# dizgotti/ouroboros-network

Measured on AMD Instinct MI355X. Metric: TPraos header verifies/sec (VRF+KES+Ed25519) at 1/2/4/8 MI355X; Ed25519 ver/s, higher is better.
Workload: dtype u32/u64 (GF(2^255-19) int limbs)

## Files before the change

### ouroboros-network_amd/csrc/devhost_vrfkey.hip

```cpp
#define OURO_NI_LINKAGE static
#include <algorithm>
#include <cstring>
#include <vector>

#include "lane_items.h"
#include "tpraos.h"
#include "vrfkey_ws.h"

using namespace ouro;

namespace {
const int32_t* host_btab() {
  static std::vector<int32_t> tab = [] {
    std::vector<int32_t> t(kBTabWords);
    build_btab(t.data());
    return t;
  }();
  return tab.data();
}
const int32_t* host_ubtab() {
  static std::vector<int32_t> tab = [] {
    std::vector<int32_t> t(kUBTabWords);
    build_ubtab(t.data());
    return t;
  }();
  return tab.data();
}
struct Lane {
  std::vector<int32_t> buf;
  Slot s;
  Lane() : buf(slot_region_words(1, kLaneWords) + 4, 0) {
    s = Slot{reinterpret_cast<int32_t*>((reinterpret_cast<uintptr_t>(buf.data()) + 15) & ~uintptr_t(15))};
  }
};
void encode_result(uint8_t* out, Slot lane) {
  const ge_p2 U = dsm_result(lane);
  uint32_t enc[8];
  ge_encode_with_inv(enc, U.X, U.Y, fe_invert(U.Z));
  memcpy(out, enc, 32);
}
}

extern "C" {

void dh_vrfkey_params(int* width, int* windows, int* entries, size_t* tab_words,
                      size_t* base_words, size_t* min_per_key) {
  *width = kYW;
  *windows = kYWindows;
  *entries = kYKeyEntries;
  *tab_words = kYKeyWords;
  *base_words = kYBaseWords;
  *min_per_key = kVrfKeyMinPerKey;
}
int dh_vrfkey_build(const uint8_t* pk, int32_t* tab, int32_t* base) {
  uint32_t p[8];
  bytes_to_words8(p, pk);
  const bool ok = vrfkey_base(p, base);
  for (int j = 0; j < kYWindows; j++) vrfkey_fill(base, tab, j);
  return ok ? 1 : 0;
}
void dh_vrfkey_u(uint8_t* out, const int32_t* tab, const uint8_t* c16, const uint8_t* s32) {
  alignas(16) uint8_t proof[80] = {0};
  memcpy(proof + 32, c16, 16);
  memcpy(proof + 48, s32, 32);
  ouro_tpraos_batch b{};
  b.n = 1;
  b.eta_proof = proof;
  Lane lane;
  std::vector<int32_t> res(kResWords + 4, 0);
  hdr_u_shared(b, 0, false, true, lane.s, Slot{res.data()}, host_ubtab(), tab);
  encode_result(out, lane.s);
}
int dh_vrfkey_u_inline(uint8_t* out, const uint8_t* pk, const uint8_t* c16, const uint8_t* s32) {
  uint32_t p[8], pi[20] = {0};
  bytes_to_words8(p, pk);
  memcpy(pi + 8, c16, 16);
  memcpy(pi + 12, s32, 32);
  Lane lane;
  const bool ok = vrf_u_core(p, pi, true, 2, lane.s, host_btab());
  encode_result(out, lane.s);
  return ok ? 1 : 0;
}
int dh_tpraos_verify_shared(const ouro_tpraos_batch* b, const int32_t* tab, int key_ok,
                            uint8_t* verdict, uint8_t* beta_eta, uint8_t* beta_leader) {
  Lane lane;
  std::vector<int32_t> rr(kResWords + 4, 0);
  const Slot r{rr.data()};
  const uint32_t opts = batch_opts(*b);
  for (size_t i = 0; i < b->n; i++) {
    std::fill(rr.begin(), rr.end(), 0);
    for (int core = 0; core < kHdrCores; core++) {
      if (core == kCoreUe || core == kCoreUl)
        hdr_u_shared(*b, i, core == kCoreUl, key_ok != 0, lane.s, r, host_ubtab(), tab);
      else
        hdr_core(*b, i, opts, core, lane.s, r, host_btab());
    }
    hdr_finish_item(*b, i, opts, r, lane.s, verdict, beta_eta, beta_leader);
  }
  return 0;
}
size_t dh_vrfkey_layout(size_t n, size_t budget, size_t* out7) {
  const VrfKeyLayout L = vrfkey_layout(n, kYKeyBytes, budget);
  const size_t v[7] = {L.kmax, L.cap, L.off_rep, L.off_uniq, L.off_kidx, L.off_flag, L.group_bytes};
  memcpy(out7, v, sizeof v);
  return L.table_bytes;
}

int dh_lt_u_table(int nkeys, const uint8_t* keys, int n, const uint32_t* kidx,
                  const uint8_t* proofs, int stride, uint32_t* out) {
  if (nkeys <= 0 || n <= 0 || stride <= 0 || !keys || !kidx || !proofs || !out) return -1;
  std::vector<int32_t> tabs((size_t)nkeys * kYKeyWords), base(kYBaseWords);
  std::vector<uint8_t> flag(nkeys);
  for (int k = 0; k < nkeys; k++)
    flag[k] = (uint8_t)dh_vrfkey_build(keys + 32 * (size_t)k, tabs.data() + (size_t)k * kYKeyWords,
                                       base.data());
  ouro_tpraos_batch b{};
  b.n = (size_t)n;
  b.eta_proof = proofs;
  for (int i = 0; i < n; i++) {
    if (kidx[i] >= (uint32_t)nkeys) return -1;
    Lane lane;
    std::vector<int32_t> res(kResWords + 4, 0);
    lt::u_table_item(b, (size_t)i, flag[kidx[i]] != 0, out + (size_t)i * lt::kChainOut, lane.s,
                     Slot{res.data()}, host_ubtab(), tabs.data() + (size_t)kidx[i] * kYKeyWords);
  }
  return 0;
}
}
```

### ouroboros-network_amd/csrc/verify.h

```cpp
#pragma once
#include <vector>

#include "blake2b.h"
#include "ge25519.h"
#include "lattice.h"
#include "modinv.h"
#include "sc25519.h"
#include "sha512.h"

namespace ouro {

constexpr int kCachedWords = 40;
constexpr int kTabEntries = 8;
constexpr int kTabWords = kTabEntries * kCachedWords;
constexpr int kSlotTab1 = 0;
constexpr int kSlotTab2 = kTabWords;
constexpr int kSlotTab3 = 2 * kTabWords;
constexpr int kSlotA1 = 3 * kTabWords;
constexpr int kSlotA2 = kSlotA1 + 8;
constexpr int kSlotB = kSlotA2 + 8;
constexpr int kSlotCarry = kSlotB + 8;
constexpr int kSlotOut = kSlotCarry + 8;
constexpr int kLaneWords = kSlotOut + 36;

#ifndef OURO_SLOT_GROUP
#define OURO_SLOT_GROUP 1
#endif
constexpr int kSlotGroup = OURO_SLOT_GROUP;
constexpr int kChunkStride = 4 * kSlotGroup;
struct Slot {
  int32_t* p;
  OURO_FI Slot operator+(int w) const {
    OURO_TRK(if (w & 3) ouro_trk_violation();)
    return Slot{p + (w >> 2) * kChunkStride};
  }
  OURO_FI Slot chunks(int k) const { return Slot{p + k * kChunkStride}; }
  OURO_FI int32_t* word(int w) const { return p + (w >> 2) * kChunkStride + (w & 3); }
  OURO_FI int4* chunk(int k) const { return reinterpret_cast<int4*>(p + k * kChunkStride); }
};
OURO_FI Slot slot_of(int32_t* base, size_t s, int slot_words) {
  return Slot{base + (s / kSlotGroup) * (size_t)kSlotGroup * slot_words + (s % kSlotGroup) * 4};
}
constexpr size_t slot_region_words(size_t n, int slot_words) {
  return (n + kSlotGroup - 1) / kSlotGroup * kSlotGroup * (size_t)slot_words;
}

#ifndef OURO_BW
#define OURO_BW 16
#endif
constexpr int kBW = OURO_BW;
constexpr int kBStride = kBW / 4;
constexpr bool kBSplitRecode = (128 % kBW) != 0;
constexpr int kBDigitsHalf = kBSplitRecode ? (128 + kBW) / kBW : 128 / kBW;
constexpr int kBTabEntries = 1 << (kBW - 1);
constexpr int kNielsWords = 32;
constexpr size_t kBTabWords = 2 * (size_t)kBTabEntries * kNielsWords;

OURO_FI void st_fe(Slot p, const fe& f) {
  stg4(p.chunk(0), make_int4(f.v[0], f.v[1], f.v[2], f.v[3]));
  stg4(p.chunk(1), make_int4(f.v[4], f.v[5], f.v[6], f.v[7]));
  stg2(p.chunk(2), make_int2(f.v[8], f.v[9]));
  OURO_TRK(ouro_trk_store(p.p, f.b));
}
OURO_FI fe ld_fe(Slot p) {
  const int4 a = ldg4(p.chunk(0)), b = ldg4(p.chunk(1));
  const int2 c = ldg2(p.chunk(2));
  fe f = fe_make(a.x, a.y, a.z, a.w, b.x, b.y, b.z, b.w, c.x, c.y);
  OURO_TRK(ouro_trk_load(p.p, f.b));
  return f;
}
OURO_FI fe ld_fe_w2(const int32_t* base, int w0, int stride) {
  int2 q[5];
#pragma unroll
  for (int j = 0; j < 5; j++) {
    const int w = w0 + 2 * j;
    q[j] = ldg2(base + (w >> 2) * stride + (w & 3));
  }
  return fe_make(q[0].x, q[0].y, q[1].x, q[1].y, q[2].x, q[2].y, q[3].x, q[3].y, q[4].x, q[4].y);
}
OURO_FI void st_cached(Slot p, const ge_cached& c) {
  const uint32_t* s[4] = {c.YplusX.v, c.YminusX.v, c.Z2.v, c.T2d.v};
  int32_t w[40];
#pragma unroll
  for (int k = 0; k < 4; k++)
#pragma unroll
    for (int i = 0; i < 10; i++) w[10 * k + i] = s[k][i];
#pragma unroll
  for (int i = 0; i < 10; i++)
    stg4(p.chunk(i), make_int4(w[4 * i], w[4 * i + 1], w[4 * i + 2], w[4 * i + 3]));
  OURO_TRK(ouro_trk_store(p.word(0), c.YplusX.b); ouro_trk_store(p.word(10), c.YminusX.b);
           ouro_trk_store(p.word(20), c.Z2.b); ouro_trk_store(p.word(30), c.T2d.b);)
}
OURO_FI ge_cached ld_cached(Slot p) {
  int32_t w[40];
#pragma unroll
  for (int i = 0; i < 10; i++) {
    int4 v = ldg4(p.chunk(i));
    w[4 * i] = v.x; w[4 * i + 1] = v.y; w[4 * i + 2] = v.z; w[4 * i + 3] = v.w;
  }
  ge_cached c;
#pragma unroll
  for (int i = 0; i < 10; i++) {
    c.YplusX.v[i] = w[i];
    c.YminusX.v[i] = w[10 + i];
    c.Z2.v[i] = w[20 + i];
    c.T2d.v[i] = w[30 + i];
  }
  OURO_TRK(ouro_trk_load(p.word(0), c.YplusX.b); ouro_trk_load(p.word(10), c.YminusX.b);
           ouro_trk_load(p.word(20), c.Z2.b); ouro_trk_load(p.word(30), c.T2d.b);)
  return c;
}
#ifndef OURO_TAB_PACK
#define OURO_TAB_PACK 1
#endif
constexpr int kPackedWords = 32;
constexpr int kLaneEntryWords = OURO_TAB_PACK ? kPackedWords : kCachedWords;
OURO_FI void fe_pack256(uint32_t w[8], const fe& f) {
  OURO_TRK(for (int i = 0; i < 10; i++) trk_check(f.b[i] < (1ull << 28));)
  uint32_t h[10];
#pragma unroll
  for (int i = 0; i < 10; i++) h[i] = f.v[i];
  uint32_t c = h[9] >> 25;
  h[9] &= limb_mask(9);
  h[0] += 19 * c;
#pragma unroll
  for (int i = 0; i < 9; i++) {
    c = h[i] >> limb_bits(i);
    h[i] &= limb_mask(i);
    h[i + 1] += c;
  }
  w[0] = h[0] | (h[1] << 26);
  w[1] = (h[1] >> 6) | (h[2] << 19);
  w[2] = (h[2] >> 13) | (h[3] << 13);
  w[3] = (h[3] >> 19) | (h[4] << 6);
  w[4] = h[5] | (h[6] << 25);
  w[5] = (h[6] >> 7) | (h[7] << 19);
  w[6] = (h[7] >> 13) | (h[8] << 12);
  w[7] = (h[8] >> 20) | (h[9] << 6);
}
OURO_FI fe fe_unpack256(const uint32_t w[8]) {
  fe h;
  h.v[0] = w[0] & 0x3ffffff;
  h.v[1] = ((w[0] >> 26) | (w[1] << 6)) & 0x1ffffff;
  h.v[2] = ((w[1] >> 19) | (w[2] << 13)) & 0x3ffffff;
  h.v[3] = ((w[2] >> 13) | (w[3] << 19)) & 0x1ffffff;
  h.v[4] = (w[3] >> 6) & 0x3ffffff;
  h.v[5] = w[4] & 0x1ffffff;
  h.v[6] = ((w[4] >> 25) | (w[5] << 7)) & 0x3ffffff;
  h.v[7] = ((w[5] >> 19) | (w[6] << 13)) & 0x1ffffff;
  h.v[8] = ((w[6] >> 12) | (w[7] << 20)) & 0x3ffffff;
  h.v[9] = w[7] >> 6;
  OURO_TRK(for (int i = 0; i < 9; i++) h.b[i] = limb_mask(i); h.b[9] = (1u << 26) - 1;)
  return h;
}
OURO_FI void st_cached_packed(Slot p, const ge_cached& c) {
  const fe* s[4] = {&c.YplusX, &c.YminusX, &c.Z2, &c.T2d};
#pragma unroll
  for (int k = 0; k < 4; k++) {
    uint32_t w[8];
    fe_pack256(w, *s[k]);
    stg4(p.chunk(2 * k), make_int4((int)w[0], (int)w[1], (int)w[2], (int)w[3]));
    stg4(p.chunk(2 * k + 1), make_int4((int)w[4], (int)w[5], (int)w[6], (int)w[7]));
  }
}
OURO_FI ge_cached ld_cached_packed(Slot p) {
  fe f[4];
#pragma unroll
  for (int k = 0; k < 4; k++) {
    const int4 a = ldg4(p.chunk(2 * k)), b = ldg4(p.chunk(2 * k + 1));
    const uint32_t w[8] = {(uint32_t)a.x, (uint32_t)a.y, (uint32_t)a.z, (uint32_t)a.w,
                           (uint32_t)b.x, (uint32_t)b.y, (uint32_t)b.z, (uint32_t)b.w};
    f[k] = fe_unpack256(w);
  }
  return ge_cached{f[0], f[1], f[2], f[3]};
}
OURO_FI void st_entry(Slot p, const ge_cached& c, bool quad) {
  if (OURO_TAB_PACK && !quad)
    st_cached_packed(p, c);
  else
    st_cached(p, c);
}
OURO_FI ge_niels ld_niels(const int32_t* p) {
  int32_t w[32];
#pragma unroll
  for (int i = 0; i < 8; i++) {
    int4 v = ldg4(p + 4 * i);
    w[4 * i] = v.x; w[4 * i + 1] = v.y; w[4 * i + 2] = v.z; w[4 * i + 3] = v.w;
  }
  ge_niels n;
#pragma unroll
  for (int i = 0; i < 10; i++) {
    n.yplusx.v[i] = w[i];
    n.yminusx.v[i] = w[10 + i];
    n.xy2d.v[i] = w[20 + i];
  }
  OURO_TRK(ouro_trk_load(p, n.yplusx.b); ouro_trk_load(p + 10, n.yminusx.b);
           ouro_trk_load(p + 20, n.xy2d.b);)
  return n;
}
OURO_FI void st_words8(Slot p, const uint32_t w[8]) {
  stg4(p.chunk(0), make_int4((int)w[0], (int)w[1], (int)w[2], (int)w[3]));
  stg4(p.chunk(1), make_int4((int)w[4], (int)w[5], (int)w[6], (int)w[7]));
}
OURO_FI void ld_words8(uint32_t w[8], Slot p) {
  const int4 a = ldg4(p.chunk(0)), b = ldg4(p.chunk(1));
  w[0] = a.x; w[1] = a.y; w[2] = a.z; w[3] = a.w;
  w[4] = b.x; w[5] = b.y; w[6] = b.z; w[7] = b.w;
}
OURO_FI uint64_t ld_carry(Slot lane, int k) { return ldg8(lane.word(kSlotCarry + 2 * k)); }
OURO_FI void st_carry(Slot lane, int k, uint64_t c) { stg8(lane.word(kSlotCarry + 2 * k), c); }
struct SlotTail {
  Slot s;
  OURO_FI uint32_t tail(uint32_t q) const {
    return ((uint32_t)ldg1(s.word((int)(q >> 2))) >> (8 * (q & 3))) & 0xffu;
  }
};

OURO_HD inline void build_table(Slot tab, const ge_p3& P, bool quad = false) {
  const int ec = (quad ? kCachedWords : kLaneEntryWords) / 4;
  ge_cached c1 = ge_p3_to_cached(P);
  st_entry(tab, c1, quad);
  ge_p3 Pk = quad ? ge_p1p1_to_p3_quad(ge_p2_dbl_quad(ge_p3_to_p2(P)))
                  : ge_p1p1_to_p3(ge_p3_dbl(P));
  st_entry(tab.chunks(ec), ge_p3_to_cached(Pk), quad);
#pragma unroll 1
  for (int k = 2; k < kTabEntries; k++) {
    Pk = quad ? ge_p1p1_to_p3_quad(ge_add_cached_quad(Pk, c1, false))
              : ge_p1p1_to_p3(ge_add_cached(Pk, c1, false));
    st_entry(tab.chunks(k * ec), ge_p3_to_cached(Pk), quad);
  }
}

OURO_FI uint64_t sc_recode_b(const uint32_t s[8]) {
  if constexpr (!kBSplitRecode) {
    return sc_recode_carries<kBW, 2 * kBDigitsHalf>(s);
  } else {
  uint64_t mask = 0;
#pragma unroll
  for (int h = 0; h < 2; h++) {
    uint32_t c = 0;
#pragma unroll
    for (int k = 0; k < kBDigitsHalf; k++) {
      const int rel = kBW * k, bit = 128 * h + rel;
      const int w = bit >> 5, sh = bit & 31;
      const uint64_t two = (uint64_t)s[w] | ((w + 1 < 8 ? (uint64_t)s[w + 1] : 0ull) << 32);
      uint32_t v = (uint32_t)(two >> sh) & ((1u << kBW) - 1);
      if (128 - rel < kBW) v &= (1u << (128 - rel)) - 1;
      mask |= (uint64_t)c << (kBDigitsHalf * h + k);
      c = (v + c) > (1u << (kBW - 1)) ? 1u : 0u;
    }
  }
  return mask;
  }
}

OURO_FI void ss_shr5(uint32_t w[5], int bits) {
#pragma unroll
  for (int i = 0; i < 4; i++) w[i] = (w[i] >> bits) | (w[i + 1] << (32 - bits));
  w[4] >>= bits;
}

constexpr uint32_t dsm_cfg(int nw1, int nw2, bool useB, int tab1 = 0, int tab2 = 1) {
  return (uint32_t)nw1 | ((uint32_t)nw2 << 8) | (useB ? (1u << 16) : 0u) |
         ((uint32_t)tab1 << 20) | ((uint32_t)tab2 << 22);
}

#ifndef OURO_DSM_SKIP_ID
#define OURO_DSM_SKIP_ID 1
#endif
#ifndef OURO_DBL_UNROLL
#define OURO_DBL_UNROLL 1
#endif
#ifndef OURO_DBL_UNROLL_QUAD
#define OURO_DBL_UNROLL_QUAD 4
#endif
#ifndef OURO_ADD_UNROLL_QUAD
#define OURO_ADD_UNROLL_QUAD 4
#endif
#ifndef OURO_PF_AT
#define OURO_PF_AT 3
#endif
#ifndef OURO_ADD_LOCKSTEP
#define OURO_ADD_LOCKSTEP 1
#endif
#ifndef OURO_DBL_LOCKSTEP
#define OURO_DBL_LOCKSTEP 1
#endif
OURO_FI ge_p1p1 dsm_dbl(const ge_p1p1& t) {
  if constexpr (OURO_DBL_LOCKSTEP) return ge_dbl_lockstep(t);
  else return ge_p2_dbl(ge_p1p1_to_p2(t));
}
template <bool kQuad>
OURO_FI void dsm_body(Slot lane, const int32_t* btab, uint32_t cfg) {
  const int nw1 = (int)(cfg & 0x7f), nw2 = (int)((cfg >> 8) & 0x7f);
  const bool useB = (cfg >> 16) & 1;
  const Slot tab1 = lane.chunks((int)((cfg >> 20) & 3) * (kTabWords / 4));
  const Slot tab2 = lane.chunks((int)((cfg >> 22) & 3) * (kTabWords / 4));
  constexpr int kE = kQuad ? kCachedWords : kLaneEntryWords;
  uint32_t a1[8], a2[8], b[8];
  ld_words8(a1, lane + kSlotA1);
  ld_words8(a2, lane + kSlotA2);
  ld_words8(b, lane + kSlotB);
  const uint64_t c1 = ld_carry(lane, 0), c2 = ld_carry(lane, 1), cb = ld_carry(lane, 2);
  int top = nw1 > nw2 ? nw1 : nw2;
  if (useB && top < kBStride * kBDigitsHalf) top = kBStride * kBDigitsHalf;
#pragma unroll 1
  for (int s = top; s < 64; s++) {
    ss_shl<8>(a1, 4);
    ss_shl<8>(a2, 4);
  }
  constexpr int kBPre = 160 - kBW * kBDigitsHalf;
  uint32_t blo[5] = {0, b[0], b[1], b[2], b[3]};
  uint32_t bhi[5] = {0, b[4], b[5], b[6], b[7]};
  if (kBPre < 32) {
    ss_shr5(blo, 32 - kBPre);
    ss_shr5(bhi, 32 - kBPre);
  }
  uint32_t prefetch = 0;
  ge_p1p1 t{fe_zero(), fe_one(), fe_one(), fe_one()};
  bool fresh = true;
#pragma unroll 1
  for (int j = top - 1; j >= 0; j--) {
    const bool act1 = j < nw1, act2 = j < nw2;
    const bool actB = useB && (j % kBStride) == 0 && j < kBStride * kBDigitsHalf;
    const bool actB2 = actB;
    int32_t d1 = 0, d2 = 0, d3 = 0, d4 = 0;
    if (act1) d1 = sc_digit_from<4>(a1[7] >> 28, c1, j, 64);
    if (act2) d2 = sc_digit_from<4>(a2[7] >> 28, c2, j, 64);
    ss_shl<8>(a1, 4);
    ss_shl<8>(a2, 4);
    if (actB) {
      const int k = j / kBStride;
      d3 = sc_digit_from<kBW>(blo[4] >> (32 - kBW), cb, k,
                              kBSplitRecode ? kBDigitsHalf : 2 * kBDigitsHalf);
      d4 = sc_digit_from<kBW>(bhi[4] >> (32 - kBW), cb, k + kBDigitsHalf, 2 * kBDigitsHalf);
      ss_shl<5>(blo, kBW);
      ss_shl<5>(bhi, kBW);
    }
    const int i1 = (d1 < 0 ? -d1 : d1) - 1, i2 = (d2 < 0 ? -d2 : d2) - 1;
    const Slot e1 = tab1.chunks((i1 > 0 ? i1 : 0) * (kE / 4));
    const Slot e2 = tab2.chunks((i2 > 0 ? i2 : 0) * (kE / 4));
    uint32_t pf1 = 0, pf2 = 0, pf3 = 0, pf4 = 0, pf5 = 0, pf6 = 0;
    const int i3 = (d3 < 0 ? -d3 : d3) - 1, i4 = (d4 < 0 ? -d4 : d4) - 1;
#define OURO_TOUCH_ENTRIES()                                                                   \
  do {                                                                                         \
    if (act1) { pf1 = (uint32_t)ldg1(e1.word(0)); if (kE > 32) pf2 = (uint32_t)ldg1(e1.word(kE - 1)); } \
    if (act2) { pf3 = (uint32_t)ldg1(e2.word(0)); if (kE > 32) pf4 = (uint32_t)ldg1(e2.word(kE - 1)); } \
    if (actB) {           \
      pf5 = (uint32_t)ldg1(btab + (size_t)(i3 > 0 ? i3 : 0) * kNielsWords);                    \
      pf6 = (uint32_t)ldg1(btab + ((size_t)kBTabEntries + (i4 > 0 ? i4 : 0)) * kNielsWords);   \
    }                                                                                          \
  } while (0)
    const bool skip_dbl = OURO_DSM_SKIP_ID && j == top - 1;
    if (kQuad || OURO_PF_AT == 0 || skip_dbl) OURO_TOUCH_ENTRIES();
    if (!skip_dbl) {
      if constexpr (kQuad) {
#pragma unroll OURO_DBL_UNROLL_QUAD
        for (int k = 0; k < 4; k++) t = ge_dbl_from_p1p1_quad(t);
      } else if (OURO_PF_AT == 0) {
#pragma unroll OURO_DBL_UNROLL
        for (int k = 0; k < 4; k++) t = dsm_dbl(t);
      } else {
#pragma unroll 1
        for (int k = 0; k < 3; k++) t = dsm_dbl(t);
        OURO_TOUCH_ENTRIES();
        t = dsm_dbl(t);
      }
    }
#undef OURO_TOUCH_ENTRIES
    prefetch ^= pf1 ^ pf2 ^ pf3 ^ pf4 ^ pf5 ^ pf6;
    constexpr int kAddUnroll = kQuad ? OURO_ADD_UNROLL_QUAD : 1;
#pragma unroll kAddUnroll
    for (int src = 0; src < 4; src++) {
      const bool active = src == 0 ? act1 : src == 1 ? act2 : src == 2 ? actB : actB2;
      if (!active) continue;
      const int32_t d = src == 0 ? d1 : src == 1 ? d2 : src == 2 ? d3 : d4;
      const bool neg = d < 0;
      const int32_t mag = neg ? -d : d;
      const int idx = mag > 0 ? mag - 1 : 0;
#if defined(__HIP_DEVICE_COMPILE__)
      if (kQuad && !(OURO_DSM_SKIP_ID && fresh)) {
        const uint32_t qp = threadIdx.x & 3u;
        const bool niels = src >= 2;
        const int k = qp < 2 ? (int)(qp ^ (neg ? 1u : 0u)) : (qp == 2 ? (niels ? 2 : 3) : (niels ? 0 : 2));
        const int32_t* ent =
            niels ? btab + ((src == 3 ? (size_t)kBTabEntries : 0) + idx) * kNielsWords
                  : (src == 0 ? tab1 : tab2).chunks(idx * (kCachedWords / 4)).p;
        fe b = ld_fe_w2(ent, 10 * k, niels ? 4 : kChunkStride);
        if (mag == 0 || (niels && qp == 3)) {
          b = fe_zero();
          b.v[0] = qp < 2 ? 1u : (qp == 2 ? 0u : 2u);
        }
        t = ge_add_own_quad(t, b, neg);
        continue;
      }
#endif
      ge_cached q;
      if (src < 2) {
        const Slot e = (src == 0 ? tab1 : tab2).chunks(idx * (kE / 4));
        q = kE == kPackedWords ? ld_cached_packed(e) : ld_cached(e);
      } else {
        const size_t base = src == 3 ? kBTabEntries : 0;
        ge_niels nq = ld_niels(btab + (base + idx) * kNielsWords);
        q = ge_cached{nq.yplusx, nq.yminusx, fe_two(), nq.xy2d};
      }
      if (mag == 0) q = ge_cached_identity();
      if (OURO_DSM_SKIP_ID && fresh) {
        const fe qa = fe_select(q.YminusX, q.YplusX, neg);
        const fe qb = fe_select(q.YplusX, q.YminusX, neg);
        t = ge_p1p1{fe_carry(fe_sub4(qa, qb)), fe_carry(fe_add(qa, qb)), q.Z2, q.Z2};
        fresh = false;
        continue;
      }
      if constexpr (kQuad) t = ge_add_cached_quad(ge_p1p1_to_p3_quad(t), q, neg);
      else if constexpr (OURO_ADD_LOCKSTEP) t = ge_add_lockstep<OURO_ADD_LOCKSTEP == 2>(t, q, neg, src >= 2);
      else t = ge_add_cached(ge_p1p1_to_p3(t), q, neg, src >= 2);
    }
  }
  ge_p2 r = kQuad ? ge_p1p1_to_p2_quad(t) : ge_p1p1_to_p2(t);
  st_fe(lane + kSlotOut, r.X);
  st_fe(lane + kSlotOut + 12, r.Y);
  st_fe(lane + kSlotOut + 24, r.Z);
  if (prefetch == 0xffffffffu) stg1(lane.word(kSlotOut + 35), (int32_t)prefetch);
}
OURO_NI void dsm_lane(Slot lane, const int32_t* btab, uint32_t cfg) {
  dsm_body<false>(lane, btab, cfg);
}
#if defined(__HIPCC__)
__device__ __noinline__ void dsm_lane_dsm_launch(Slot lane, const int32_t* btab, uint32_t cfg) {
  dsm_body<false>(lane, btab, cfg);
}
#endif
OURO_NI void dsm_quad(Slot lane, const int32_t* btab, uint32_t cfg) {
  dsm_body<true>(lane, btab, cfg);
}
OURO_FI void dsm(Slot lane, const int32_t* btab, uint32_t cfg, bool quad = false) {
  if (quad)
    dsm_quad(lane, btab, cfg);
  else
    dsm_lane(lane, btab, cfg);
}

OURO_FI ge_p2 dsm_result(Slot lane) {
  return ge_p2{ld_fe(lane + kSlotOut), ld_fe(lane + kSlotOut + 12), ld_fe(lane + kSlotOut + 24)};
}

#ifndef OURO_YW
#define OURO_YW 6
#endif
constexpr int kYW = OURO_YW;
static_assert(kYW >= 4 && kYW <= 8, "OURO_YW: 4 .. 8");
constexpr int kYWindows = (128 + kYW) / kYW;
constexpr int kYWinEntries = 1 << (kYW - 1);
constexpr int kYTopEntries = (1 << (128 - kYW * (kYWindows - 1))) - 1 + 1;
static_assert(kYTopEntries <= kYWinEntries, "the top window's digits fit a window");
constexpr int kYKeyEntries = (kYWindows - 1) * kYWinEntries + kYTopEntries;
constexpr size_t kYKeyWords = (size_t)kYKeyEntries * kPackedWords;
constexpr int kYBasePtWords = 48;
constexpr size_t kYBaseWords = (size_t)kYWindows * kYBasePtWords;
constexpr size_t kYKeyBytes = 4 * (kYKeyWords + kYBaseWords);

OURO_FI void st_fe_at(int32_t* p, const fe& f) {
  stg4(p, make_int4(f.v[0], f.v[1], f.v[2], f.v[3]));
  stg4(p + 4, make_int4(f.v[4], f.v[5], f.v[6], f.v[7]));
  stg2(p + 8, make_int2(f.v[8], f.v[9]));
  OURO_TRK(ouro_trk_store(p, f.b));
}
OURO_FI fe ld_fe_at(const int32_t* p) {
  const int4 a = ldg4(p), b = ldg4(p + 4);
  const int2 c = ldg2(p + 8);
  fe f = fe_make(a.x, a.y, a.z, a.w, b.x, b.y, b.z, b.w, c.x, c.y);
  OURO_TRK(ouro_trk_load(p, f.b));
  return f;
}
OURO_FI void st_cached_packed_at(int32_t* p, const ge_cached& c) {
  const fe* s[4] = {&c.YplusX, &c.YminusX, &c.Z2, &c.T2d};
#pragma unroll
  for (int k = 0; k < 4; k++) {
    uint32_t w[8];
    fe_pack256(w, *s[k]);
    stg4(p + 8 * k, make_int4((int)w[0], (int)w[1], (int)w[2], (int)w[3]));
    stg4(p + 8 * k + 4, make_int4((int)w[4], (int)w[5], (int)w[6], (int)w[7]));
  }
}
OURO_FI ge_cached ld_cached_packed_at(const int32_t* p) {
  fe f[4];
#pragma unroll
  for (int k = 0; k < 4; k++) {
    const int4 a = ldg4(p + 8 * k), b = ldg4(p + 8 * k + 4);
    const uint32_t w[8] = {(uint32_t)a.x, (uint32_t)a.y, (uint32_t)a.z, (uint32_t)a.w,
                           (uint32_t)b.x, (uint32_t)b.y, (uint32_t)b.z, (uint32_t)b.w};
    f[k] = fe_unpack256(w);
  }
  return ge_cached{f[0], f[1], f[2], f[3]};
}

OURO_HD inline bool vrfkey_base(const uint32_t pk[8], int32_t* base) {
  ge_p3 Y;
  bool ok = !ge_has_small_order(pk) && ge_is_canonical(pk);
  ok = ge_decode(&Y, pk, false) && ok;
  ge_p3 P = ge_p3_neg(Y);
#pragma unroll 1
  for (int j = 0; j < kYWindows; j++) {
    int32_t* b = base + j * kYBasePtWords;
    st_fe_at(b, P.X);
    st_fe_at(b + 12, P.Y);
    st_fe_at(b + 24, P.Z);
    st_fe_at(b + 36, P.T);
    if (j + 1 == kYWindows) break;
    ge_p1p1 t = ge_p3_dbl(P);
#pragma unroll 1
    for (int k = 1; k < kYW; k++) t = dsm_dbl(t);
    P = ge_p1p1_to_p3(t);
  }
  return ok;
}
OURO_FI int vrfkey_win_entries(int j) { return j + 1 < kYWindows ? kYWinEntries : kYTopEntries; }
OURO_FI size_t vrfkey_win_word(int j) { return (size_t)j * kYWinEntries * kPackedWords; }
OURO_HD inline void vrfkey_fill(const int32_t* base, int32_t* tab, int j) {
  const int32_t* b = base + j * kYBasePtWords;
  const ge_p3 P{ld_fe_at(b), ld_fe_at(b + 12), ld_fe_at(b + 24), ld_fe_at(b + 36)};
  int32_t* e = tab + vrfkey_win_word(j);
  const int n = vrfkey_win_entries(j);
  const ge_cached c1 = ge_p3_to_cached(P);
  st_cached_packed_at(e, c1);
  if (n < 2) return;
  ge_p3 Pk = ge_p1p1_to_p3(ge_p3_dbl(P));
  st_cached_packed_at(e + kPackedWords, ge_p3_to_cached(Pk));
#pragma unroll 1
  for (int m = 2; m < n; m++) {
    Pk = ge_p1p1_to_p3(ge_add_cached(Pk, c1, false));
    st_cached_packed_at(e + m * kPackedWords, ge_p3_to_cached(Pk));
  }
}

OURO_FI void ss_shr4(uint32_t w[4], int bits) {
#pragma unroll
  for (int i = 0; i < 3; i++) w[i] = (w[i] >> bits) | (w[i + 1] << (32 - bits));
  w[3] >>= bits;
}

OURO_FI void ss_shr8(uint32_t w[8], int bits) {
#pragma unroll
  for (int i = 0; i < 7; i++) w[i] = (w[i] >> bits) | (w[i + 1] << (32 - bits));
  w[7] >>= bits;
}

#ifndef OURO_UBW
#define OURO_UBW 12
#endif
constexpr int kUBW = OURO_UBW;
static_assert(kUBW >= 8 && kUBW <= 16, "OURO_UBW: 8 .. 16");
constexpr int kUBDigits = (253 + kUBW) / kUBW;
constexpr int kUBWinEntries = 1 << (kUBW - 1);
constexpr size_t kUBTabWords = (size_t)kUBDigits * kUBWinEntries * kNielsWords;

OURO_NI void vrf_u_fixed_lane(Slot lane, const int32_t* ubtab, const int32_t* ytab) {
  uint32_t a[8], b[8];
  ld_words8(a, lane + kSlotA1);
  ld_words8(b, lane + kSlotB);
  uint32_t c[4] = {a[0], a[1], a[2], a[3]};
  constexpr uint32_t kYMask = (1u << kYW) - 1u, kBMask = (1u << kUBW) - 1u;
  constexpr int kTrips = kYWindows > kUBDigits ? kYWindows : kUBDigits;
  uint32_t cy = 0, cbw = 0;
  auto next_y = [&]() {
    const uint32_t v = (c[0] & kYMask) + cy;
    ss_shr4(c, kYW);
    cy = v > (1u << (kYW - 1)) ? 1u : 0u;
    return (int32_t)v - (int32_t)(cy << kYW);
  };
  auto next_b = [&]() {
    const uint32_t v = (b[0] & kBMask) + cbw;
    ss_shr8(b, kUBW);
    cbw = v > (1u << (kUBW - 1)) ? 1u : 0u;
    return (int32_t)v - (int32_t)(cbw << kUBW);
  };
  auto y_entry = [&](int j, int32_t d) {
    const int mag = d < 0 ? -d : d;
    return ytab + vrfkey_win_word(j) + (size_t)(mag > 0 ? mag - 1 : 0) * kPackedWords;
  };
  auto b_entry = [&](int j, int32_t d) {
    const int mag = d < 0 ? -d : d;
    return ubtab + ((size_t)j * kUBWinEntries + (mag > 0 ? mag - 1 : 0)) * kNielsWords;
  };
  int32_t dy = next_y(), db = next_b();
  uint32_t prefetch = 0;
  ge_p1p1 t{fe_zero(), fe_one(), fe_one(), fe_one()};
  bool fresh = true;
#pragma unroll 1
  for (int j = 0; j < kTrips; j++) {
    const bool actB = j < kUBDigits, actY = j < kYWindows;
    int32_t ny = 0, nb = 0;
#pragma unroll 1
    for (int src = 0; src < 2; src++) {
      if (!(src == 0 ? actB : actY)) continue;
      const int32_t d = src == 0 ? db : dy;
      const bool neg = d < 0;
      ge_cached q;
      if (src == 0) {
        const ge_niels nq = ld_niels(b_entry(j, d));
        q = ge_cached{nq.yplusx, nq.yminusx, fe_two(), nq.xy2d};
      } else {
        q = ld_cached_packed_at(y_entry(j, d));
      }
      if (src == 1 || !actY) {
        if (j + 1 < kYWindows) {
          ny = next_y();
          prefetch ^= (uint32_t)ldg1(y_entry(j + 1, ny));
        }
        if (j + 1 < kUBDigits) {
          nb = next_b();
          prefetch ^= (uint32_t)ldg1(b_entry(j + 1, nb));
        }
      }
      if (d == 0) q = ge_cached_identity();
      if (fresh) {
        const fe qa = fe_select(q.YminusX, q.YplusX, neg);
        const fe qb = fe_select(q.YplusX, q.YminusX, neg);
        t = ge_p1p1{fe_carry(fe_sub4(qa, qb)), fe_carry(fe_add(qa, qb)), q.Z2, q.Z2};
        fresh = false;
        continue;
      }
      t = ge_add_lockstep<false>(t, q, neg, src == 0);
    }
    dy = ny;
    db = nb;
  }
  const ge_p2 r = ge_p1p1_to_p2(t);
  st_fe(lane + kSlotOut, r.X);
  st_fe(lane + kSlotOut + 12, r.Y);
  st_fe(lane + kSlotOut + 24, r.Z);
  if (prefetch == 0xffffffffu) stg1(lane.word(kSlotOut + 35), (int32_t)prefetch);
}

enum Phase { kPhaseAll = 0, kPhasePre = 1, kPhasePost = 2 };
constexpr int kSlotCfg = kSlotCarry + 6;
OURO_FI void dsm_or_defer(Slot lane, const int32_t* btab, uint32_t cfg, bool quad, int phase) {
  if (phase == kPhasePre) {
    stg1(lane.word(kSlotCfg), (int32_t)cfg);
    return;
  }
  dsm(lane, btab, cfg, quad);
}
OURO_FI bool dsm_result_is_identity(Slot lane) {
  const ge_p2 Q = dsm_result(lane);
  return fe_iszero(Q.X) && fe_iszero(fe_sub(Q.Y, Q.Z));
}

OURO_FI int wave_max_small(int x) {
#if defined(__HIP_DEVICE_COMPILE__)
  int m = 0;
#pragma unroll
  for (int b = 6; b >= 0; b--) {
    const int trial = m | (1 << b);
    if (__ballot(x >= trial) != 0) m = trial;
  }
  return m;
#else
  return x;
#endif
}

OURO_HD inline void ed25519_scalars_from_digest(HalfScalars& hs, uint32_t b[8], const uint64_t H[8],
                                                const uint32_t S[8]);
template <class Tail>
OURO_HD inline void ed25519_scalars(HalfScalars& hs, uint32_t b[8], const uint32_t R[8],
                                    const uint32_t S[8], const uint32_t pk[8], const Tail& msg,
                                    uint32_t mlen) {
  uint32_t pre[16];
#pragma unroll
  for (int i = 0; i < 8; i++) {
    pre[i] = R[i];
    pre[8 + i] = pk[i];
  }
  uint64_t H[8];
  sha512_prefixed<64>(H, pre, msg, mlen);
  ed25519_scalars_from_digest(hs, b, H, S);
}
OURO_HD inline void ed25519_scalars_from_digest(HalfScalars& hs, uint32_t b[8], const uint64_t H[8],
                                                const uint32_t S[8]) {
  uint32_t hw[16], h[8];
  sha512_digest_words(hw, H);
  sc_reduce512(h, hw);
  ed25519_half_scalars(hs, h);
  uint32_t prod[16];
#pragma unroll
  for (int i = 0; i < 16; i++) prod[i] = 0;
#pragma unroll
  for (int i = 0; i < 8; i++) {
    uint64_t carry = 0;
#pragma unroll
    for (int j = 0; j < 8; j++) {
      const uint64_t t = (uint64_t)hs.c1[i] * S[j] + prod[i + j] + carry;
      prod[i + j] = (uint32_t)t;
      carry = t >> 32;
    }
    prod[i + 8] = (uint32_t)carry;
  }
  sc_reduce512(b, prod);
}

OURO_FI bool ed25519_precheck(const uint32_t R[8], const uint32_t S[8], const uint32_t pk[8],
                              bool byron) {
  if (byron) return (S[7] >> 29) == 0;
  bool ok = sc_is_canonical(S) && !ge_has_small_order(R);
  return ok && ge_is_canonical(pk) && !ge_has_small_order(pk);
}

template <class Tail>
OURO_HD inline bool ed25519_verify_lane(const uint32_t sig[16], const uint32_t pk[8],
                                        const Tail& msg, uint32_t mlen, Slot lane,
                                        const int32_t* btab, bool byron = false,
                                        bool quad = false, int phase = kPhaseAll) {
  if (phase == kPhasePost) return dsm_result_is_identity(lane);
  uint32_t R[8], S[8];
#pragma unroll
  for (int i = 0; i < 8; i++) {
    R[i] = sig[i];
    S[i] = sig[8 + i];
  }
  bool ok = ed25519_precheck(R, S, pk, byron);
  ge_p3 negA, negR;
  bool okA, okR;
  if (quad) {
    ge_decode_pair_quad(&negA, &okA, &negR, &okR, pk, R, true);
  } else {
    ge_decode_pair(&negA, &okA, &negR, &okR, pk, R, true);
  }
  ok = okA && ok;
  ok = ge_is_canonical(R) && ok;
  ok = okR && ok;
  ok = ok && !(fe_iszero(negR.X) && (R[7] >> 31) != 0);
  HalfScalars hs;
  uint32_t b[8];
  ed25519_scalars(hs, b, R, S, pk, msg, mlen);
  build_table(lane + kSlotTab1, hs.c0_neg ? ge_p3_neg(negA) : negA, quad);
  build_table(lane + kSlotTab2, negR, quad);
  st_words8(lane + kSlotA1, hs.c0);
  st_words8(lane + kSlotA2, hs.c1);
  st_words8(lane + kSlotB, b);
  st_carry(lane, 0, sc_recode_carries<4, 64>(hs.c0));
  st_carry(lane, 1, sc_recode_carries<4, 64>(hs.c1));
  st_carry(lane, 2, sc_recode_b(b));
  int nw = wave_max_small((hs.bits + 4) >> 2);
  nw = nw < 1 ? 1 : (nw > 64 ? 64 : nw);
  dsm_or_defer(lane, btab, dsm_cfg(nw, nw, true, 0, 1), quad, phase);
  if (phase == kPhasePre) return ok;
  return ok && dsm_result_is_identity(lane);
}

struct Ell2Pre {
  fe rr, r2, D, num, W, W3;
};
OURO_HD inline fe elligator2_pre(Ell2Pre& e, const uint32_t r[8]) {
  e.rr = fe_from_words(r);
  e.r2 = fe_sq(e.rr);
  e.D = fe_carry(fe_add(fe_add(e.r2, e.r2), fe_one()));
  fe A2r2 = fe_mul(fe_mont_a2(), e.r2);
  e.W = fe_carry(fe_sub4(fe_sq(e.D), fe_add(A2r2, A2r2)));
  e.num = fe_mul(fe_mont_a2a(), e.D);
  e.W3 = fe_mul(fe_sq(e.W), e.W);
  const fe W7 = fe_mul(fe_sq(e.W3), e.W);
  return fe_mul(e.num, W7);
}
template <bool kMul8 = true>
OURO_HD inline ge_p3 elligator2_post(const Ell2Pre& e, const fe& pw) {
  const fe A = fe_mont_a();
  const fe rr = e.rr, r2 = e.r2, D = e.D, W = e.W, num = e.num;
  fe beta = fe_mul(fe_mul(num, e.W3), pw);
  fe vxx = fe_mul(fe_sq(beta), W);
  const bool lam_p1 = fe_iszero(fe_sub4(vxx, num));
  const bool lam_m1 = fe_iszero(fe_add(vxx, num));
  const bool lam_pi = fe_iszero(fe_sub4(vxx, fe_mul(num, fe_sqrtm1())));
  const bool nonsq = !(lam_p1 || lam_m1);
  const fe F = fe_select(fe_select(fe_one_minus_i(), fe_one_plus_i(), lam_pi),
                         fe_select(fe_one(), fe_sqrtm1(), lam_p1), nonsq);
  fe x = fe_mul(beta, F);
  x = fe_select(fe_mul(x, rr), x, nonsq);
  x = fe_select(fe_neg(x), x, fe_isnegative(x));
  fe Ar2 = fe_mul(A, r2);
  fe Xn = fe_carry(fe_select(fe_neg4(fe_add(Ar2, Ar2)), fe_neg(A), nonsq));
  fe n = fe_sub(Xn, D), m = fe_add(Xn, D);
  const fe nc = fe_carry(n);
  ge_p3 P{fe_mul(x, m), nc, m, fe_mul(x, nc)};
  if constexpr (!kMul8) return P;
  return ge_mul8(P);
}
template <class Pow, bool kMul8 = true>
OURO_HD inline ge_p3 elligator2_h_with(const uint32_t r[8], Pow pow22523) {
  Ell2Pre e;
  const fe base = elligator2_pre(e, r);
  return elligator2_post<kMul8>(e, pow22523(base));
}
OURO_HD inline ge_p3 elligator2_h(const uint32_t r[8]) {
  return elligator2_h_with(r, [](const fe& z) { return fe_pow22523(z); });
}

OURO_HD inline ge_p3 elligator2_h_ref(const uint32_t r[8]) {
  const fe one = fe_one();
  const fe A = fe_mont_a();
  fe rr = fe_from_words(r);
  fe den = fe_add(fe_sq2(rr), one);
  fe x = fe_neg(fe_mul(A, fe_invert(den)));
  fe x2 = fe_sq(x);
  fe e = fe_carry(fe_add(fe_add(fe_mul(x, x2), x), fe_mul(x2, A)));
  fe chi = fe_mul(fe_sq(fe_sq(fe_pow22523(e))), fe_sq(e));
  uint32_t cw[8];
  fe_to_words(cw, chi);
  const bool e_is_minus_1 = (cw[0] >> 8) & 1;
  x = fe_carry(fe_select(fe_sub(fe_neg(x), A), x, e_is_minus_1));
  fe yed = fe_mul(fe_sub(x, one), fe_invert(fe_add(x, one)));
  uint32_t yw[8];
  fe_to_words(yw, yed);
  ge_p3 P;
  ge_decode(&P, yw, false);
  return ge_mul8(P);
}

OURO_FI void fe_invert4(fe out[4], const fe z[4]) {
  fe a1 = fe_mul(z[0], z[1]);
  fe a2 = fe_mul(a1, z[2]);
  fe a3 = fe_mul(a2, z[3]);
  fe inv = fe_invert_vartime(a3);
  out[3] = fe_mul(inv, a2);
  inv = fe_mul(inv, z[3]);
  out[2] = fe_mul(inv, a1);
  inv = fe_mul(inv, z[2]);
  out[1] = fe_mul(inv, z[0]);
  out[0] = fe_mul(inv, z[1]);
}

template <class Tail>
OURO_HD inline bool vrf03_verify_lane(uint32_t beta[16], const uint32_t pk[8],
                                      const uint32_t pi[20], const Tail& alpha, uint32_t alen,
                                      Slot lane, const int32_t* btab) {
  uint32_t G[8], c[8], s_raw[8], s[8];
#pragma unroll
  for (int i = 0; i < 8; i++) {
    G[i] = pi[i];
    s_raw[i] = pi[12 + i];
    c[i] = i < 4 ? pi[8 + i] : 0u;
  }
  ge_p3 Y, Gamma;
  bool okY, okG;
  ge_decode_pair(&Y, &okY, &Gamma, &okG, pk, G, false);
  bool ok = !ge_has_small_order(pk) && ge_is_canonical(pk);
  ok = okY && ok;
  ok = ge_is_canonical(G) && ok;
  ok = okG && ok;
  sc_reduce256(s, s_raw);
  uint32_t pre[9];
  pre[0] = 0x04u | (0x01u << 8) | (pk[0] << 16);
#pragma unroll
  for (int i = 1; i < 8; i++) pre[i] = (pk[i - 1] >> 16) | (pk[i] << 16);
  pre[8] = pk[7] >> 16;
  uint64_t Hs[8];
  sha512_prefixed<34>(Hs, pre, alpha, alen);
  uint32_t rw[16];
  sha512_digest_words(rw, Hs);
  rw[7] &= 0x7fffffffu;
  ge_p3 Hp = elligator2_h(rw);
  build_table(lane + kSlotTab1, ge_p3_neg(Y));
  st_words8(lane + kSlotA1, c);
  st_words8(lane + kSlotB, s);
  st_carry(lane, 0, sc_recode_carries<4, 33>(c));
  st_carry(lane, 2, sc_recode_b(s));
  dsm(lane, btab, dsm_cfg(33, 0, true));
  ge_p2 U = dsm_result(lane);
  build_table(lane + kSlotTab1, Hp);
  build_table(lane + kSlotTab2, ge_p3_neg(Gamma));
  st_words8(lane + kSlotA1, s);
  st_words8(lane + kSlotA2, c);
  st_carry(lane, 0, sc_recode_carries<4, 64>(s));
  st_carry(lane, 1, sc_recode_carries<4, 33>(c));
  dsm(lane, btab, dsm_cfg(64, 33, false));
  ge_p2 V = dsm_result(lane);
  ge_p3 G8 = ge_mul8(Gamma);
  fe z[4] = {Hp.Z, U.Z, V.Z, G8.Z}, zi[4];
  fe_invert4(zi, z);
  uint32_t Henc[8], Uenc[8], Venc[8], G8enc[8], Genc[8];
  ge_encode_with_inv(Henc, Hp.X, Hp.Y, zi[0]);
  ge_encode_with_inv(Uenc, U.X, U.Y, zi[1]);
  ge_encode_with_inv(Venc, V.X, V.Y, zi[2]);
  ge_encode_with_inv(G8enc, G8.X, G8.Y, zi[3]);
#pragma unroll
  for (int i = 0; i < 8; i++) Genc[i] = G[i];
  if (fe_iszero(Gamma.X)) Genc[7] &= 0x7fffffffu;
  uint32_t hp[33];
  hp[0] = 0x04u | (0x02u << 8) | (Henc[0] << 16);
#pragma unroll
  for (int i = 1; i < 8; i++) hp[i] = (Henc[i - 1] >> 16) | (Henc[i] << 16);
  hp[8] = (Henc[7] >> 16) | (Genc[0] << 16);
#pragma unroll
  for (int i = 1; i < 8; i++) hp[8 + i] = (Genc[i - 1] >> 16) | (Genc[i] << 16);
  hp[16] = (Genc[7] >> 16) | (Uenc[0] << 16);
#pragma unroll
  for (int i = 1; i < 8; i++) hp[16 + i] = (Uenc[i - 1] >> 16) | (Uenc[i] << 16);
  hp[24] = (Uenc[7] >> 16) | (Venc[0] << 16);
#pragma unroll
  for (int i = 1; i < 8; i++) hp[24 + i] = (Venc[i - 1] >> 16) | (Venc[i] << 16);
  hp[32] = Venc[7] >> 16;
  uint64_t Hc[8];
  sha512_prefixed<130>(Hc, hp, ShaNoTail{}, 0);
  uint32_t cw[16];
  sha512_digest_words(cw, Hc);
  bool ceq = true;
#pragma unroll
  for (int i = 0; i < 4; i++) ceq = ceq && cw[i] == c[i];
  ok = ok && ceq;
  uint32_t bp[9];
  bp[0] = 0x04u | (0x03u << 8) | (G8enc[0] << 16);
#pragma unroll
  for (int i = 1; i < 8; i++) bp[i] = (G8enc[i - 1] >> 16) | (G8enc[i] << 16);
  bp[8] = G8enc[7] >> 16;
  uint64_t Hb[8];
  sha512_prefixed<34>(Hb, bp, ShaNoTail{}, 0);
  uint32_t bw[16];
  sha512_digest_words(bw, Hb);
#pragma unroll
  for (int i = 0; i < 16; i++) beta[i] = ok ? bw[i] : 0u;
  return ok;
}

OURO_HD inline bool sum6kes_walk(uint32_t cur[8], uint32_t sig[16], const uint32_t vk[8],
                                 uint32_t t, const uint32_t* sigw) {
#pragma unroll
  for (int i = 0; i < 8; i++) cur[i] = vk[i];
  bool ok = true;
#pragma unroll 1
  for (int k = 6; k >= 1; k--) {
    const uint32_t* pair = sigw + 16 + 16 * (k - 1);
    uint32_t pw[16], h[8];
#pragma unroll
    for (int i = 0; i < 4; i++) {
      const int4 v = ldg4(pair + 4 * i);
      pw[4 * i] = v.x; pw[4 * i + 1] = v.y; pw[4 * i + 2] = v.z; pw[4 * i + 3] = v.w;
    }
    blake2b256_64(h, pw);
#pragma unroll
    for (int i = 0; i < 8; i++) ok = ok && h[i] == cur[i];
    const uint32_t half = 1u << (k - 1);
    const bool right = t >= half;
    t = right ? t - half : t;
#pragma unroll
    for (int i = 0; i < 8; i++) cur[i] = right ? pw[8 + i] : pw[i];
  }
#pragma unroll
  for (int i = 0; i < 4; i++) {
    const int4 v = ldg4(sigw + 4 * i);
    sig[4 * i] = v.x; sig[4 * i + 1] = v.y; sig[4 * i + 2] = v.z; sig[4 * i + 3] = v.w;
  }
  return ok;
}

template <class Tail>
OURO_HD inline bool sum6kes_verify_lane(const uint32_t vk[8], uint32_t t, const uint32_t* sigw,
                                        const Tail& msg, uint32_t mlen, Slot lane,
                                        const int32_t* btab, bool quad = false,
                                        int phase = kPhaseAll) {
  if (phase == kPhasePost) return dsm_result_is_identity(lane);
  uint32_t cur[8], sig[16];
  const bool ok = sum6kes_walk(cur, sig, vk, t, sigw);
  const bool leaf = ed25519_verify_lane(sig, cur, msg, mlen, lane, btab, false, quad, phase);
  return ok && leaf;
}

inline void build_btab_one(int32_t* out, const ge_p3& G, int entries = kBTabEntries) {
  constexpr int kChunk = 256;
  std::vector<ge_p3> pts(kChunk);
  std::vector<fe> pre(kChunk);
  ge_p3 P = G;
  for (int k0 = 0; k0 < entries; k0 += kChunk) {
    const int n = entries - k0 < kChunk ? entries - k0 : kChunk;
    for (int i = 0; i < n; i++) {
      if (k0 + i > 0) P = ge_p3_add(P, G);
      pts[i] = P;
      pre[i] = i ? fe_mul(pre[i - 1], P.Z) : P.Z;
    }
    fe inv = fe_invert(pre[n - 1]);
    for (int i = n - 1; i >= 0; i--) {
      const fe zi = i ? fe_mul(inv, pre[i - 1]) : inv;
      if (i) inv = fe_mul(inv, pts[i].Z);
      fe x = fe_mul(pts[i].X, zi), y = fe_mul(pts[i].Y, zi);
      fe yp = fe_carry(fe_add(y, x)), ym = fe_carry(fe_sub(y, x));
      fe xy2d = fe_mul(fe_mul(x, y), fe_d2());
      int32_t* e = out + (size_t)(k0 + i) * kNielsWords;
      for (int l = 0; l < 10; l++) {
        e[l] = yp.v[l];
        e[10 + l] = ym.v[l];
        e[20 + l] = xy2d.v[l];
      }
      OURO_TRK(ouro_trk_store(e, yp.b); ouro_trk_store(e + 10, ym.b); ouro_trk_store(e + 20, xy2d.b);)
      e[30] = 0;
      e[31] = 0;
    }
  }
}

inline void build_btab(int32_t* out) {
  uint32_t by[8];
  for (int i = 0; i < 8; i++) by[i] = 0x66666666u;
  by[0] = 0x66666658u;
  ge_p3 B;
  ge_decode(&B, by, false);
  build_btab_one(out, B);
  ge_p3 B128 = B;
  for (int i = 0; i < 128; i++) B128 = ge_p1p1_to_p3(ge_p3_dbl(B128));
  build_btab_one(out + (size_t)kBTabEntries * kNielsWords, B128);
}

inline void build_ubtab(int32_t* out) {
  uint32_t by[8];
  for (int i = 0; i < 8; i++) by[i] = 0x66666666u;
  by[0] = 0x66666658u;
  ge_p3 G;
  ge_decode(&G, by, false);
  for (int k = 0; k < kUBDigits; k++) {
    build_btab_one(out + (size_t)k * kUBWinEntries * kNielsWords, G, kUBWinEntries);
    for (int i = 0; i < kUBW; i++) G = ge_p1p1_to_p3(ge_p3_dbl(G));
  }
}

constexpr int kBWideU16 = 48;
constexpr size_t kBTabWideWords = (size_t)kBTabEntries * kBWideU16;
inline void build_btab_wide(uint16_t* out, const int32_t* niels) {
  for (size_t e = 0; e < 2 * (size_t)kBTabEntries; e++) {
    const int32_t* q = niels + e * kNielsWords;
    for (int k = 0; k < 3; k++) {
      const int32_t* c = q + (k == 0 ? 10 : (k == 1 ? 0 : 20));
      const fe f = fe_make(c[0], c[1], c[2], c[3], c[4], c[5], c[6], c[7], c[8], c[9]);
      uint32_t w[8];
      fe_to_words(w, f);
      for (int j = 0; j < 16; j++)
        out[e * kBWideU16 + 16 * k + j] = (uint16_t)((w[j >> 1] >> (16 * (j & 1))) & 0xffffu);
    }
  }
}

}
```

Baseline: 22.47 million.

## Store per-key VRF tables as affine Niels points with batched inversion

Per-key VRF window tables change from packed projective cached points to affine Niels points (y+x, y-x, 2dxy). Normalisation uses a Montgomery batch inversion per window. The device main loop can then use the cheaper mixed addition (Z=1) for the Y source as well as the base table, with one shared load path and no 256-bit unpacking. In exchange the per-key table build costs more, and each entry grows from packed 32 words to 32 unpacked words, which may change cache behaviour.

```diff
diff --git a/ouroboros-network_amd/csrc/devhost_vrfkey.hip b/ouroboros-network_amd/csrc/devhost_vrfkey.hip
--- a/ouroboros-network_amd/csrc/devhost_vrfkey.hip
+++ b/ouroboros-network_amd/csrc/devhost_vrfkey.hip
@@ -58,6 +58,25 @@
   const bool ok = vrfkey_base(p, base);
   for (int j = 0; j < kYWindows; j++) vrfkey_fill(base, tab, j);
   return ok ? 1 : 0;
+}
+int dh_lt_vrfkey_tables(int nkeys, const uint8_t* keys, int32_t* tabs, uint8_t* flags) {
+  if (nkeys <= 0 || nkeys > 256 || !keys || !tabs || !flags) return -1;
+  std::vector<int32_t> base(kYBaseWords);
+  for (int k = 0; k < nkeys; k++)
+    flags[k] = (uint8_t)dh_vrfkey_build(keys + 32 * (size_t)k, tabs + (size_t)k * kYKeyWords,
+                                        base.data());
+  return 0;
+}
+int dh_vrfkey_fill_point(const uint8_t* xyzt, int n, int32_t* out) {
+  if (!xyzt || !out || n < 1 || n > kYWinEntries) return -1;
+  fe c[4];
+  for (int k = 0; k < 4; k++) {
+    uint32_t w[8];
+    bytes_to_words8(w, xyzt + 32 * k);
+    c[k] = fe_from_words(w);
+  }
+  vrfkey_fill_point(ge_p3{c[0], c[1], c[2], c[3]}, out, n);
+  return 0;
 }
 void dh_vrfkey_u(uint8_t* out, const int32_t* tab, const uint8_t* c16, const uint8_t* s32) {
   alignas(16) uint8_t proof[80] = {0};
diff --git a/ouroboros-network_amd/csrc/verify.h b/ouroboros-network_amd/csrc/verify.h
--- a/ouroboros-network_amd/csrc/verify.h
+++ b/ouroboros-network_amd/csrc/verify.h
@@ -455,7 +455,7 @@
 constexpr int kYTopEntries = (1 << (128 - kYW * (kYWindows - 1))) - 1 + 1;
 static_assert(kYTopEntries <= kYWinEntries, "the top window's digits fit a window");
 constexpr int kYKeyEntries = (kYWindows - 1) * kYWinEntries + kYTopEntries;
-constexpr size_t kYKeyWords = (size_t)kYKeyEntries * kPackedWords;
+constexpr size_t kYKeyWords = (size_t)kYKeyEntries * kNielsWords;
 constexpr int kYBasePtWords = 48;
 constexpr size_t kYBaseWords = (size_t)kYWindows * kYBasePtWords;
 constexpr size_t kYKeyBytes = 4 * (kYKeyWords + kYBaseWords);
@@ -473,26 +473,19 @@
   OURO_TRK(ouro_trk_load(p, f.b));
   return f;
 }
-OURO_FI void st_cached_packed_at(int32_t* p, const ge_cached& c) {
-  const fe* s[4] = {&c.YplusX, &c.YminusX, &c.Z2, &c.T2d};
-#pragma unroll
-  for (int k = 0; k < 4; k++) {
-    uint32_t w[8];
-    fe_pack256(w, *s[k]);
-    stg4(p + 8 * k, make_int4((int)w[0], (int)w[1], (int)w[2], (int)w[3]));
-    stg4(p + 8 * k + 4, make_int4((int)w[4], (int)w[5], (int)w[6], (int)w[7]));
-  }
-}
-OURO_FI ge_cached ld_cached_packed_at(const int32_t* p) {
-  fe f[4];
-#pragma unroll
-  for (int k = 0; k < 4; k++) {
-    const int4 a = ldg4(p + 8 * k), b = ldg4(p + 8 * k + 4);
-    const uint32_t w[8] = {(uint32_t)a.x, (uint32_t)a.y, (uint32_t)a.z, (uint32_t)a.w,
-                           (uint32_t)b.x, (uint32_t)b.y, (uint32_t)b.z, (uint32_t)b.w};
-    f[k] = fe_unpack256(w);
-  }
-  return ge_cached{f[0], f[1], f[2], f[3]};
+OURO_FI void st_niels(int32_t* p, const fe& a, const fe& b, const fe& c) {
+  int32_t w[32];
+#pragma unroll
+  for (int i = 0; i < 10; i++) {
+    w[i] = (int32_t)a.v[i];
+    w[10 + i] = (int32_t)b.v[i];
+    w[20 + i] = (int32_t)c.v[i];
+  }
+  w[30] = w[31] = 0;
+#pragma unroll
+  for (int i = 0; i < 8; i++)
+    stg4(p + 4 * i, make_int4(w[4 * i], w[4 * i + 1], w[4 * i + 2], w[4 * i + 3]));
+  OURO_TRK(ouro_trk_store(p, a.b); ouro_trk_store(p + 10, b.b); ouro_trk_store(p + 20, c.b);)
 }
 
 OURO_HD inline bool vrfkey_base(const uint32_t pk[8], int32_t* base) {
@@ -516,22 +509,35 @@
   return ok;
 }
 OURO_FI int vrfkey_win_entries(int j) { return j + 1 < kYWindows ? kYWinEntries : kYTopEntries; }
-OURO_FI size_t vrfkey_win_word(int j) { return (size_t)j * kYWinEntries * kPackedWords; }
+OURO_FI size_t vrfkey_win_word(int j) { return (size_t)j * kYWinEntries * kNielsWords; }
+OURO_HD inline void vrfkey_fill_point(const ge_p3& P, int32_t* e, int n) {
+  fe pre[kYWinEntries];
+  const ge_cached c1 = ge_p3_to_cached(P);
+  ge_p3 Pk = P;
+#pragma unroll 1
+  for (int m = 0; m < n; m++) {
+    if (m == 1) Pk = ge_p1p1_to_p3(ge_p3_dbl(P));
+    if (m > 1) Pk = ge_p1p1_to_p3(ge_add_cached(Pk, c1, false));
+    const bool z0 = fe_iszero(Pk.Z);
+    const fe Z = fe_select(fe_one(), Pk.Z, z0);
+    st_niels(e + m * kNielsWords, fe_select(fe_zero(), Pk.X, z0), fe_select(fe_one(), Pk.Y, z0), Z);
+    pre[m] = m ? fe_mul(pre[m - 1], Z) : Z;
+  }
+  fe inv = fe_invert_vartime(pre[n - 1]);
+#pragma unroll 1
+  for (int m = n - 1; m >= 0; m--) {
+    const ge_niels q = ld_niels(e + m * kNielsWords);
+    const fe zi = m ? fe_mul(inv, pre[m - 1]) : inv;
+    if (m) inv = fe_mul(inv, q.xy2d);
+    const fe x = fe_mul(q.yplusx, zi), y = fe_mul(q.yminusx, zi);
+    st_niels(e + m * kNielsWords, fe_carry(fe_add(y, x)), fe_carry(fe_sub(y, x)),
+             fe_mul(fe_mul(x, y), fe_d2()));
+  }
+}
 OURO_HD inline void vrfkey_fill(const int32_t* base, int32_t* tab, int j) {
   const int32_t* b = base + j * kYBasePtWords;
   const ge_p3 P{ld_fe_at(b), ld_fe_at(b + 12), ld_fe_at(b + 24), ld_fe_at(b + 36)};
-  int32_t* e = tab + vrfkey_win_word(j);
-  const int n = vrfkey_win_entries(j);
-  const ge_cached c1 = ge_p3_to_cached(P);
-  st_cached_packed_at(e, c1);
-  if (n < 2) return;
-  ge_p3 Pk = ge_p1p1_to_p3(ge_p3_dbl(P));
-  st_cached_packed_at(e + kPackedWords, ge_p3_to_cached(Pk));
-#pragma unroll 1
-  for (int m = 2; m < n; m++) {
-    Pk = ge_p1p1_to_p3(ge_add_cached(Pk, c1, false));
-    st_cached_packed_at(e + m * kPackedWords, ge_p3_to_cached(Pk));
-  }
+  vrfkey_fill_point(P, tab + vrfkey_win_word(j), vrfkey_win_entries(j));
 }
 
 OURO_FI void ss_shr4(uint32_t w[4], int bits) {
@@ -577,7 +583,7 @@
   };
   auto y_entry = [&](int j, int32_t d) {
     const int mag = d < 0 ? -d : d;
-    return ytab + vrfkey_win_word(j) + (size_t)(mag > 0 ? mag - 1 : 0) * kPackedWords;
+    return ytab + vrfkey_win_word(j) + (size_t)(mag > 0 ? mag - 1 : 0) * kNielsWords;
   };
   auto b_entry = [&](int j, int32_t d) {
     const int mag = d < 0 ? -d : d;
@@ -596,13 +602,8 @@
       if (!(src == 0 ? actB : actY)) continue;
       const int32_t d = src == 0 ? db : dy;
       const bool neg = d < 0;
-      ge_cached q;
-      if (src == 0) {
-        const ge_niels nq = ld_niels(b_entry(j, d));
-        q = ge_cached{nq.yplusx, nq.yminusx, fe_two(), nq.xy2d};
-      } else {
-        q = ld_cached_packed_at(y_entry(j, d));
-      }
+      const ge_niels nq = ld_niels(src == 0 ? b_entry(j, d) : y_entry(j, d));
+      ge_cached q{nq.yplusx, nq.yminusx, fe_two(), nq.xy2d};
       if (src == 1 || !actY) {
         if (j + 1 < kYWindows) {
           ny = next_y();
@@ -621,7 +622,7 @@
         fresh = false;
         continue;
       }
-      t = ge_add_lockstep<false>(t, q, neg, src == 0);
+      t = ge_add_lockstep<false>(t, q, neg, true);
     }
     dy = ny;
     db = nb;
```

New measurement: 22.59 million (median of 6 runs). About the same (+0.5%).
